# ubc-vision/StableKeypoints

Measured on AMD Instinct MI355X. Metric: images/sec for token-optimization step (SD1.5, 512^2, K=10 kpts), higher is better.
Workload: dtype f32 (fp32 MFMA / VALU throughout; flash attention of the >= 1024-key self-attention layers: 3xbf16 operand split, fp32 accumulate, error <= the fp32 kernel's)

## Files before the change

### include/skp.h

```cpp
#ifndef SKP_H
#define SKP_H

#include <stdint.h>

#ifdef __cplusplus
extern "C" {
#endif

#define SKP_MAX_LAYERS 8
#define SKP_MAX_SUBJECTS 4

#define SKP_E_BADARG (-1)
#define SKP_E_RANGE  (-2)
#define SKP_E_LDS    (-3)

int skp_abi_version(void);

int skp_tune_set(const char* key, int value);
int skp_tune_get(const char* key);

int skp_gemm_nt_f32(const float* A, const float* B, float* C, int M, int N, int K, int Z0, int Z1,
                    int64_t sa0, int64_t sa1, int64_t sam, int64_t sak,
                    int64_t sb0, int64_t sb1, int64_t sbn, int64_t sbk,
                    int64_t sc0, int64_t sc1, int64_t scm, float alpha, void* stream);
// ... 102 lines not shown

int skp_add_layer_norm_ok(int C);
int skp_add_layer_norm_fwd_f32(const float* d, const float* h, const float* gamma, const float* beta, float* x, float* n,
                               float* stat, int64_t rows, int C, float eps, void* stream);
int skp_add_layer_norm_bwd_f32(const float* dn, const float* dskip, const float* x, const float* stat, const float* gamma,
                               float* dx, int64_t rows, int C, void* stream);

int skp_conv3x3_filter_f32(const void* w, void* U, int Cout, int Cin, int flip_transpose, void* stream);
int64_t skp_conv3x3_workspace(int B, int Cin, int Cout, int H, int W, int variant);
int skp_conv3x3_f32(const void* x, const void* U, const void* bias, const void* residual, void* y, void* workspace,
                    int B, int Cin, int Cout, int H, int W, int variant, void* stream);

int skp_conv3x3_f4_filter_f32(const void* w, void* U, int Cout, int Cin, int flip_transpose, void* stream);
int64_t skp_conv3x3_f4_workspace(int B, int Cin, int Cout, int H, int W);
int skp_conv3x3_f4_f32(const void* x, const void* U, const void* bias, const void* residual, void* y, void* workspace,
                       int B, int Cin, int Cout, int H, int W, void* stream);

int skp_conv3x3_f4_stats_blocks(int B, int Cin, int Cout, int H, int W);
int skp_conv3x3_f4_stats_f32(const void* x, const void* U, const void* bias, const void* residual, void* y, float* stats,
                             int B, int Cin, int Cout, int H, int W, void* stream);
int skp_conv3x3_s2_stats_f32(const void* x, const void* U, const void* bias, void* y, float* stats, int B, int Cin, int Cout,
                             int H, int W, int pad, void* stream);
int skp_group_norm_fwd_blocks_f32(const float* x, const float* off, const float* gamma, const float* beta, float* y,
                                  float* mean, float* rstd, const float* bs, int nblk, int pix, int N, int C, int G, int HW,
                                  float eps, int silu, void* stream);

int skp_conv3x3_s2_filter_f32(const void* w, void* U, int Cout, int Cin, void* stream);
int skp_conv3x3_s2_f32(const void* x, const void* U, const void* bias, void* y, int B, int Cin, int Cout, int H, int W,
                       int pad, void* stream);
int64_t skp_conv3x3_s2_workspace(int B, int Cin, int Cout, int H, int W);
int skp_conv3x3_s2_ws_f32(const void* x, const void* U, const void* bias, void* y, void* workspace, int B, int Cin, int Cout,
                          int H, int W, int pad, void* stream);

int skp_conv3x3_small_f32(const void* x, const void* w, const void* bias, void* y, int B, int Cin, int Cout, int H, int W,
                          void* stream);
int skp_conv3x3_small_stats_blocks(int B, int Cin, int Cout, int H, int W);
int skp_conv3x3_small_stats_f32(const void* x, const void* w, const void* bias, void* y, float* stats, int B, int Cin, int Cout,
                                int H, int W, void* stream);

int skp_geglu_fwd_f32(const float* p, float* y, int64_t rows, int inner, void* stream);
int skp_geglu_bwd_f32(const float* p, const float* dy, float* dp, int64_t rows, int inner, void* stream);

int skp_nchw_to_tokens_f32(const float* x, float* y, int B, int C, int HW, void* stream);
int skp_tokens_to_nchw_f32(const float* t, const float* residual, float* y, int B, int C, int HW, void* stream);

int skp_token_stats_f32(const float* M, int T, int R, int num_subjects, float sigma, float eps,
                        int32_t* argmax, float* kl, float* entropy, void* stream);

int skp_select_tokens(const float* kl, const int32_t* argmax_t, int T, int R, int n_cand, int top_k,
                      int64_t* cand, int64_t* sel, void* stream);
int skp_select_tokens_batched(const float* kl, const int32_t* argmax_t, int n, int T, int R, int n_cand, int top_k,
                              int64_t* cand, int64_t* sel, void* stream);

int skp_losses_fwd_f32(const float* M, const float* Mt, const int64_t* sel, int K, int T, int R,
                       const int32_t* argmax, int num_subjects, float sigma,
                       const float* theta_inv , float* partial, float* g_sharp,
                       float* g_eq_a, float* g_eq_b, void* stream);
int skp_losses_fwd_dev_f32(const float* M, const float* Mt, const int64_t* sel, int K, int T, int R,
                           const int32_t* argmax, int num_subjects, float sigma, const float* theta_inv_dev,
                           float* partial, float* g_sharp, float* g_eq_a, float* g_eq_b, void* stream);

int skp_rows_axpy_f32(float* dst, const int64_t* sel, int K, int64_t n, const float* x, const float* a,
                      const float* y, const float* b, void* stream);

#ifdef __cplusplus
}
// ... 3 lines not shown
```

### stablekeypoints_amd/_native.py

```python
from __future__ import annotations

import ctypes as C
import os

import torch

_HERE = os.path.dirname(os.path.abspath(__file__))
LIB_PATH = os.environ.get("SKP_LIB_PATH") or os.path.join(_HERE, "csrc", "libskp_hip.so")
ABI_VERSION = 39

_vp, _i, _f, _i64 = C.c_void_p, C.c_int, C.c_float, C.c_int64

SIGNATURES = {
    "skp_abi_version": [],
    "skp_tune_set": [C.c_char_p, _i],
    "skp_tune_get": [C.c_char_p],
    "skp_group_norm_onepass_ok": [_i, _i, _i, _i],
    "skp_gemm_nt_f32": [_vp, _vp, _vp, _i, _i, _i, _i, _i,
                        _i64, _i64, _i64, _i64, _i64, _i64, _i64, _i64, _i64, _i64, _i64, _f, _vp],
    "skp_qk_logits_f32": [_vp, _vp, _vp, _i, _i, _i, _i, _i, _i, _f, _vp],
    "skp_attn_map_fwd_f32": [C.POINTER(_vp), C.POINTER(_i), _i, _i, _i, _i, _i, _vp, _vp, _vp],
    "skp_attn_map_fwd_ex_f32": [C.POINTER(_vp), C.POINTER(_i), _i, _i, _i, _i, _i, _vp, _vp, _vp, _i, _i64, _i, _vp],
    "skp_attn_map_bwd_ex_f32": [C.POINTER(_vp), C.POINTER(_vp), C.POINTER(_i), _i, _i, _i, _i, _i, _vp, _vp, _vp, _vp,
                                _i, _i64, _i, _vp],
    "skp_attn_map_bwd_workspace": [C.POINTER(_i), _i, _i, _i, _i, _i],
    "skp_attn_map_bwd_f32": [C.POINTER(_vp), C.POINTER(_vp), C.POINTER(_i), _i, _i, _i, _i, _i, _vp, _vp, _vp, _vp],
    "skp_group_norm_coef_f32": [_vp, _vp, _vp, _vp, _vp, _vp, _vp, _vp, _i, _i, _vp, _i, _i, _i, _i, _f, _vp],
    "skp_conv3x3_f4_gn_ok": [_i, _i, _i, _i, _i],
    "skp_conv3x3_f4_gn_f32": [_vp, _vp, _vp, _vp, _vp, _vp, _vp, _i, _i, _i, _i, _i, _vp],
    "skp_unwarp_accumulate_f32": [_vp, _vp, _i, _i, _i, _i, _vp, _vp, _i, _vp],
    "skp_attn_map_fwd_wide_f32": [C.POINTER(_vp), C.POINTER(_i), _i, _i, _i, _i, _i, _vp, _vp, _vp, _i, _i, _vp],
    "skp_attn_map_fwd_wide_ok": [C.POINTER(_i), _i, _i, _i],
    "skp_attn_map_bwd_col_ok": [C.POINTER(_i), _i, _i, _i, _i, _i],
    "skp_attn_map_bwd_col_workspace": [C.POINTER(_i), _i, _i, _i, _i, _i, _i],
    "skp_attn_map_bwd_col_f32": [C.POINTER(_vp), C.POINTER(_vp), C.POINTER(_i), _i, _i, _i, _i, _i, _vp, _vp, _i, _vp, _vp,
                                 _i, _vp],
    "skp_attn_map_bwd_sparse_workspace": [C.POINTER(_i), _i, _i, _i, _i, _i, _i],
    "skp_attn_map_bwd_sparse_f32": [C.POINTER(_vp), C.POINTER(_vp), C.POINTER(_i), _i, _i, _i, _i, _i, _vp, _vp, _i, _vp, _vp,
                                    _i, _vp],
    "skp_token_stats_f32": [_vp, _i, _i, _i, _f, _f, _vp, _vp, _vp, _vp],
    "skp_select_tokens": [_vp, _vp, _i, _i, _i, _i, _vp, _vp, _vp],
    "skp_select_tokens_batched": [_vp, _vp, _i, _i, _i, _i, _i, _vp, _vp, _vp],
# ... 1 lines not shown
    "skp_losses_fwd_dev_f32": [_vp, _vp, _vp, _i, _i, _i, _vp, _i, _f, _vp, _vp, _vp, _vp, _vp, _vp],
    "skp_rows_axpy_f32": [_vp, _vp, _i, _i64, _vp, _vp, _vp, _vp, _vp],
    "skp_cross_attn_fwd_f32": [_vp, _vp, _vp, _vp, _vp, _i, _i, _i, _i, _i, _i, _f, _vp],
    "skp_cross_attn_bwd_workspace": [_i, _i, _i, _i, _i],
    "skp_cross_attn_bwd_f32": [_vp, _vp, _vp, _vp, _vp, _vp, _vp, _vp, _vp, _vp, _i, _i, _i, _i, _i, _i, _f, _vp],
    "skp_group_norm_fwd_f32": [_vp, _vp, _vp, _vp, _vp, _vp, _vp, _vp, _i, _i, _i, _i, _f, _i, _vp],
    "skp_group_norm_bwd_f32": [_vp, _vp, _vp, _vp, _vp, _vp, _vp, _vp, _vp, _i, _i, _i, _i, _f, _i, _vp],
    "skp_group_norm_bwd_add_f32": [_vp, _vp, _vp, _vp, _vp, _vp, _vp, _vp, _vp, _vp, _i, _i, _i, _i, _f, _i, _vp],
    "skp_add_bias_residual_f32": [_vp, _vp, _vp, _vp, _i, _i, _i, _vp],
    "skp_add_layer_norm_ok": [_i],
    "skp_add_layer_norm_fwd_f32": [_vp, _vp, _vp, _vp, _vp, _vp, _vp, _i64, _i, _f, _vp],
    "skp_add_layer_norm_bwd_f32": [_vp, _vp, _vp, _vp, _vp, _vp, _i64, _i, _vp],
    "skp_conv3x3_filter_f32": [_vp, _vp, _i, _i, _i, _vp],
    "skp_conv3x3_workspace": [_i, _i, _i, _i, _i, _i],
    "skp_conv3x3_f32": [_vp, _vp, _vp, _vp, _vp, _vp, _i, _i, _i, _i, _i, _i, _vp],
    "skp_conv3x3_f4_filter_f32": [_vp, _vp, _i, _i, _i, _vp],
    "skp_conv3x3_f4_workspace": [_i, _i, _i, _i, _i],
    "skp_conv3x3_f4_f32": [_vp, _vp, _vp, _vp, _vp, _vp, _i, _i, _i, _i, _i, _vp],
    "skp_flash_attn_fwd_split_ok": [_i, _i, _i, _i, _i, _i],
    "skp_flash_attn_fwd_split_workspace": [_i, _i, _i, _i, _i, _i],
    "skp_flash_attn_fwd_split_f32": [_vp, _vp, _vp, _vp, _vp, _vp, _i, _i, _i, _i, _i, _i, C.c_float, _vp],
    "skp_flash_attn_bwd_split_ok": [_i, _i, _i, _i, _i, _i],
    "skp_flash_attn_bwd_split_workspace": [_i, _i, _i, _i, _i, _i],
    "skp_flash_attn_bwd_split_f32": [_vp, _vp, _vp, _vp, _vp, _vp, _vp, _vp, _vp, _vp, _i, _i, _i, _i, _i, _i, _f, _vp],
    "skp_flash_attn_bwd_split_ld_f32": [_vp, _vp, _vp, _vp, _vp, _vp, _vp, _vp, _vp, _vp, _i, _i, _i, _i, _i, _i, _f, _i, _vp],
    "skp_conv3x3_f4r_ok": [_i, _i, _i, _i, _i],
    "skp_conv3x3_f4r_filter_f32": [_vp, _vp, _i, _i, _i, _vp],
    "skp_conv3x3_f4r_workspace": [_i, _i, _i, _i, _i],
    "skp_conv3x3_f4r_f32": [_vp, _vp, _vp, _vp, _vp, _vp, _i, _i, _i, _i, _i, _vp],
    "skp_conv3x3_s2_filter_f32": [_vp, _vp, _i, _i, _vp],
    "skp_conv3x3_s2_f32": [_vp, _vp, _vp, _vp, _i, _i, _i, _i, _i, _i, _vp],
    "skp_conv3x3_s2_workspace": [_i, _i, _i, _i, _i],
    "skp_conv3x3_s2_ws_f32": [_vp, _vp, _vp, _vp, _vp, _i, _i, _i, _i, _i, _i, _vp],
    "skp_conv3x3_small_f32": [_vp, _vp, _vp, _vp, _i, _i, _i, _i, _i, _vp],
    "skp_conv3x3_small_stats_blocks": [_i, _i, _i, _i, _i],
    "skp_conv3x3_small_stats_f32": [_vp, _vp, _vp, _vp, _vp, _i, _i, _i, _i, _i, _vp],
    "skp_conv3x3_f4_stats_blocks": [_i, _i, _i, _i, _i],
    "skp_conv3x3_f4_stats_f32": [_vp, _vp, _vp, _vp, _vp, _vp, _i, _i, _i, _i, _i, _vp],
    "skp_conv3x3_s2_stats_f32": [_vp, _vp, _vp, _vp, _vp, _i, _i, _i, _i, _i, _i, _vp],
    "skp_group_norm_fwd_blocks_f32": [_vp, _vp, _vp, _vp, _vp, _vp, _vp, _vp, _i, _i, _i, _i, _i, _i, _f, _i, _vp],
    "skp_geglu_fwd_f32": [_vp, _vp, _i64, _i, _vp],
    "skp_geglu_bwd_f32": [_vp, _vp, _vp, _i64, _i, _vp],
    "skp_nchw_to_tokens_f32": [_vp, _vp, _i, _i, _i, _vp],
    "skp_tokens_to_nchw_f32": [_vp, _vp, _vp, _i, _i, _i, _vp],
    "skp_flash_attn_fwd_f32": [_vp, _vp, _vp, _vp, _vp, _i, _i, _i, _i, _i, _i, _f, _vp],
    "skp_flash_attn_bwd_workspace": [_i, _i, _i, _i, _i, _i],
    "skp_flash_attn_bwd_f32": [_vp, _vp, _vp, _vp, _vp, _vp, _vp, _vp, _vp, _vp, _i, _i, _i, _i, _i, _i, _f, _vp],
    "skp_flash_attn_bwd_ld_f32": [_vp, _vp, _vp, _vp, _vp, _vp, _vp, _vp, _vp, _vp, _i, _i, _i, _i, _i, _i, _f, _i, _vp],
    "skp_self_attn_fwd_f32": [_vp, _vp, _vp, _vp, _vp, _i, _i, _i, _i, _f, _vp],
    "skp_self_attn_bwd_f32": [_vp, _vp, _vp, _vp, _vp, _vp, _vp, _vp, _vp, _vp, _i, _i, _i, _i, _f, _vp],
}

_ERR = {-1: "SKP_E_BADARG (null pointer / non-positive size)",
        -2: "SKP_E_RANGE (size outside the built kernel range)",
        -3: "SKP_E_LDS (tile exceeds 160 KiB LDS)"}

_lib = None


class NativeLibraryError(RuntimeError):
    pass


def lib():
    global _lib
    if _lib is not None:
# ... 65 lines not shown
```

### stablekeypoints_amd/csrc/skp_common.h

```cpp
#pragma once
#include <hip/hip_runtime.h>
#include <stdint.h>
#include "../../include/skp.h"

#define SKP_WAVE 64
#define SKP_LOG2E 1.4426950408889634f

typedef float f32x16 __attribute__((ext_vector_type(16)));
typedef float f32x4 __attribute__((ext_vector_type(4)));
typedef float f32x2 __attribute__((ext_vector_type(2)));

enum { SKP_TUNE_WINO_SPLIT = 0, SKP_TUNE_WINO_RAW_MAX_TILES, SKP_TUNE_MAP_BANDS, SKP_TUNE_FA2_TWO_KERNEL_BWD, SKP_TUNE_GN_FOLD_MAX_COUT, SKP_TUNE_CROSS_ATTN_TS,
       SKP_TUNE_COUNT };
int skp_tune(int key);

static inline int skp_launch_status() {
    hipError_t e = hipGetLastError();
    return e == hipSuccess ? 0 : (int)e;
}

__device__ __forceinline__ void skp_cubic_taps(int dst, float ratio, int n, int idx[4], float w[4]) {
    const float A = -0.75f;
    const float src = ratio * ((float)dst + 0.5f) - 0.5f;
    const float fl = floorf(src);
    const float t = src - fl;
    const int i0 = (int)fl;
    float x = t + 1.0f;
    w[0] = ((A * x - 5.0f * A) * x + 8.0f * A) * x - 4.0f * A;
    x = t;
    w[1] = ((A + 2.0f) * x - (A + 3.0f)) * x * x + 1.0f;
    x = 1.0f - t;
    w[2] = ((A + 2.0f) * x - (A + 3.0f)) * x * x + 1.0f;
    x = 2.0f - t;
    w[3] = ((A * x - 5.0f * A) * x + 8.0f * A) * x - 4.0f * A;
#pragma unroll
    for (int i = 0; i < 4; ++i) {
        int v = i0 - 1 + i;
        idx[i] = v < 0 ? 0 : (v > n - 1 ? n - 1 : v);
    }
}

__device__ __forceinline__ float skp_wave_sum(float v) {
#pragma unroll
    for (int o = 32; o > 0; o >>= 1) v += __shfl_xor(v, o, 64);
    return v;
}
// ... 34 lines not shown
```

### stablekeypoints_amd/csrc/skp_select_loss.hip

```cpp
#include "skp_common.h"
#include <string.h>

__device__ __forceinline__ bool skp_better(float v, int i, float bv, int bi) {
    return (v > bv) || (v == bv && i < bi);
}

struct StatsArgs { int T, R, S; float sigma, eps; };

__global__ __launch_bounds__(256) void skp_token_stats_kernel(const float* __restrict__ M, StatsArgs a,
                                                              int32_t* __restrict__ argmax_out,
                                                              float* __restrict__ kl_out, float* __restrict__ ent_out) {
    __shared__ float red_v[4];
    __shared__ int red_i[4];
    __shared__ float red[4];
    __shared__ float s_cy[SKP_MAX_SUBJECTS], s_cx[SKP_MAX_SUBJECTS];
    const int t = blockIdx.x, tid = threadIdx.x, R = a.R, RR = R * R;
    const float* m = M + (size_t)t * RR;
    const float rad = 0.05f * (float)R;
    const float rad2 = rad * rad;
    float maxval0 = 0.f;
    for (int j = 0; j < a.S; ++j) {
        float bv = -INFINITY; int bi = 0x7fffffff;
        for (int p = tid; p < RR; p += 256) {
            const int row = p / R, col = p - row * R;
// ... 338 lines not shown
                                  const int32_t* argmax, int num_subjects, float sigma, const float* theta_inv,
                                  float* partial, float* g_sharp, float* g_eq_a, float* g_eq_b, void* stream) {
    return losses_run(M, Mt, sel, K, T, R, argmax, num_subjects, sigma, theta_inv, nullptr, partial, g_sharp, g_eq_a, g_eq_b, stream);
}

extern "C" int skp_losses_fwd_dev_f32(const float* M, const float* Mt, const int64_t* sel, int K, int T, int R,
                                      const int32_t* argmax, int num_subjects, float sigma, const float* theta_inv_dev,
                                      float* partial, float* g_sharp, float* g_eq_a, float* g_eq_b, void* stream) {
    if (!theta_inv_dev) return SKP_E_BADARG;
    return losses_run(M, Mt, sel, K, T, R, argmax, num_subjects, sigma, nullptr, theta_inv_dev, partial, g_sharp, g_eq_a, g_eq_b, stream);
}

__global__ __launch_bounds__(256) void skp_rows_axpy_kernel(float* __restrict__ dst, const int64_t* __restrict__ sel,
                                                            int64_t n, const float* __restrict__ x,
                                                            const float* __restrict__ a, const float* __restrict__ y,
                                                            const float* __restrict__ b) {
    const int k = blockIdx.y;
    const int64_t i = (int64_t)blockIdx.x * 256 + threadIdx.x;
    if (i >= n) return;
    float v = a[0] * x[(size_t)k * n + i];
    if (y) v += b[0] * y[(size_t)k * n + i];
    dst[(size_t)sel[k] * n + i] += v;
}

extern "C" int skp_rows_axpy_f32(float* dst, const int64_t* sel, int K, int64_t n, const float* x, const float* a,
                                 const float* y, const float* b, void* stream) {
    if (!dst || !sel || !x || !a || K <= 0 || n <= 0 || (y && !b)) return SKP_E_BADARG;
    if (K > 65535) return SKP_E_RANGE;
    hipLaunchKernelGGL(skp_rows_axpy_kernel, dim3((unsigned)((n + 255) / 256), K), dim3(256), 0, (hipStream_t)stream,
                       dst, sel, n, x, a, y, b);
    return skp_launch_status();
}

extern "C" int skp_abi_version(void) { return 39; }

static int g_tune[SKP_TUNE_COUNT] = {0};
static const char* const g_tune_names[SKP_TUNE_COUNT] = {"wino_split", "wino_raw_max_tiles", "map_bands", "fa2_two_kernel_bwd", "gn_fold_max_cout", "cross_attn_ts"};
int skp_tune(int key) { return (key >= 0 && key < SKP_TUNE_COUNT) ? g_tune[key] : 0; }
extern "C" int skp_tune_set(const char* key, int value) {
    if (!key || value < 0) return SKP_E_BADARG;
    for (int i = 0; i < SKP_TUNE_COUNT; ++i)
        if (!strcmp(key, g_tune_names[i])) { g_tune[i] = value; return 0; }
    return SKP_E_RANGE;
}
extern "C" int skp_tune_get(const char* key) {
    if (!key) return SKP_E_BADARG;
    for (int i = 0; i < SKP_TUNE_COUNT; ++i)
        if (!strcmp(key, g_tune_names[i])) return g_tune[i];
    return SKP_E_RANGE;
}
```

### stablekeypoints_amd/ops.py

```python
from __future__ import annotations

import contextlib
import weakref
from typing import List, Sequence, Tuple

import torch

from . import _native as N
from . import routes


def _stream() -> int:
    return torch.cuda.current_stream().cuda_stream


def _dev(t: torch.Tensor, name: str) -> torch.Tensor:
    if not t.is_cuda:
        raise RuntimeError(f"{name}: the StableKeypoints hot path runs on the HIP kernels only "
                           f"(got a {t.device} tensor; there is no CPU fallback)")
    if t.dtype != torch.float32:
        raise RuntimeError(f"{name}: expected float32, got {t.dtype}")
    return t if t.is_contiguous() else t.contiguous()


# ... 794 lines not shown
    def backward(ctx, gx, gn):
        x, stat, weight = ctx.saved_tensors
        C = x.shape[-1]
        if gn is None:
            dx = gx
        else:
            gn = _dev(gn, "gn")
            gx = _dev(gx, "gx") if gx is not None else None
            dx = torch.empty_like(x)
            N.check(N.lib().skp_add_layer_norm_bwd_f32(gn.data_ptr(), gx.data_ptr() if gx is not None else None, x.data_ptr(),
                                                       stat.data_ptr(), weight.data_ptr(), dx.data_ptr(), x.numel() // C, C,
                                                       _stream()), "skp_add_layer_norm_bwd_f32")
        return (dx if ctx.has_d else None), dx, None, None, None


def add_layer_norm(d, h, norm: torch.nn.LayerNorm):
    routes.note("add_layer_norm", "add_ln")
    return AddLayerNormFn.apply(d, h, norm.weight, norm.bias, norm.eps)


def conv3x3_supported(x_shape, w_shape, need_grad=True):
    if len(w_shape) != 4 or tuple(w_shape[2:]) != (3, 3) or len(x_shape) != 4:
        return False
    co, ci = int(w_shape[0]), int(w_shape[1])
    if co % 32 or ci % 32:
        return False
    _, _, h, w = (int(v) for v in x_shape)
    return max(ci * h * w, co * h * w, 16 * ci * co) * 4 < 2 ** 31


_FILTER_FORMS = {"f2": ("skp_conv3x3_filter_f32", 16),
                 "f4": ("skp_conv3x3_f4_filter_f32", 36),
                 "f4r": ("skp_conv3x3_f4r_filter_f32", 9),
                 "s2": ("skp_conv3x3_s2_filter_f32", 9)}


def _filters(weight, form, backward=False):
    def build():
        w = _dev(weight.detach(), "weight")
        co, ci = w.shape[:2]
        name, per_pair = _FILTER_FORMS[form]
        U = torch.empty(per_pair * co * ci, device=w.device, dtype=torch.float32)
        if form == "s2":
            N.check(N.lib().skp_conv3x3_s2_filter_f32(w.data_ptr(), U.data_ptr(), co, ci, _stream()), name)
        else:
            N.check(getattr(N.lib(), name)(w.data_ptr(), U.data_ptr(), *((ci, co, 1) if backward else (co, ci, 0)), _stream()), name)
        return U
    return cached(weight, ("filters", form, bool(backward)), (weight,), build)


def _wino_filters(weight, backward):
    return _filters(weight, "f2", backward)


def _wino4_filters(weight, backward):
    return _filters(weight, "f4", backward)


def _wino4r_filters(weight, backward):
    return _filters(weight, "f4r", backward)


def _conv3x3_raw(x, U, bias, cout, variant=0, split=True, residual=None, out=None):
    B, ci, H, W = x.shape
    y = out if out is not None else torch.empty(B, cout, H, W, device=x.device, dtype=torch.float32)
    ws = _workspace("skp_conv3x3_workspace", B, ci, cout, H, W, int(variant), device=x.device) if split else None
    N.check(N.lib().skp_conv3x3_f32(x.data_ptr(), U.data_ptr(), _ptr(bias), _ptr(residual), y.data_ptr(), _ptr(ws),
                                    B, ci, cout, H, W, int(variant), _stream()), "skp_conv3x3_f32")
    return y


def _conv3x3_f4_raw(x, U, bias, cout, split=True, residual=None, out=None, stats=None):
    B, ci, H, W = x.shape
    y = out if out is not None else torch.empty(B, cout, H, W, device=x.device, dtype=torch.float32)
    if stats is not None:
        N.check(N.lib().skp_conv3x3_f4_stats_f32(x.data_ptr(), U.data_ptr(), _ptr(bias), _ptr(residual), y.data_ptr(),
                                                 stats.data_ptr(), B, ci, cout, H, W, _stream()), "skp_conv3x3_f4_stats_f32")
# ... 352 lines not shown
        ctx.weight = weight
        ctx.xshape, ctx.pad = tuple(x.shape), int(pad)
        return _conv3x3_s2_raw(x, weight, bias, pad, False)

    @staticmethod
    def backward(ctx, dy):
        w = ctx.weight
        b, c, h, wd = ctx.xshape
        co = w.shape[0]
        if S2_BWD_OWN and h % 2 == 0 and wd % 2 == 0 and conv3x3_wanted((b, co, h, wd), (c, co, 3, 3)):
            dy = _dev(dy, "dy")
            routes.note("conv3x3_s2.bwd_data", "zero_stuffed")
            up = torch.zeros(b, co, h, wd, device=dy.device, dtype=torch.float32)
            o = 0 if ctx.pad == 1 else 1
            up[:, :, o::2, o::2] = dy
            return _conv3x3_run(up, w, True, None, None, c), None, None, None
        routes.note("conv3x3_s2.bwd_data", "lib")
        if ctx.pad == 1:
            return torch.nn.grad.conv2d_input(ctx.xshape, w, dy.contiguous(), stride=2, padding=1), None, None, None
        dxp = torch.nn.grad.conv2d_input((b, c, h + 1, wd + 1), w, dy.contiguous(), stride=2, padding=0)
        return dxp[:, :, :h, :wd], None, None, None


def conv3x3_s2(x, weight, bias=None, pad: int = 0, want_stats: bool = False):
    if weight.requires_grad or (bias is not None and bias.requires_grad):
        raise RuntimeError("conv3x3_s2: frozen weights only")
    if torch.is_grad_enabled() and x.requires_grad:
        return ConvS2Fn.apply(x, weight, bias, int(pad))
    return _conv3x3_s2_raw(x, weight, bias, pad, want_stats)


def _conv3x3_s2_raw(x, weight, bias, pad, want_stats):
    x = _dev(x.detach(), "x")
    routes.note("conv3x3_s2", "s2_direct")
    U = _filters(weight, "s2")
    B, ci, H, W = x.shape
    co = weight.shape[0]
    y = torch.empty(B, co, H // 2, W // 2, device=x.device, dtype=torch.float32)
    if want_stats and GN_FUSED_STATS:
        nblk = (H // 16) * (W // 32)
        stats = torch.empty(B, co, nblk, 2, device=x.device, dtype=torch.float32)
        N.check(N.lib().skp_conv3x3_s2_stats_f32(x.data_ptr(), U.data_ptr(), _ptr(bias), y.data_ptr(), stats.data_ptr(),
                                                 B, ci, co, H, W, int(pad), _stream()), "skp_conv3x3_s2_stats_f32")
        y._skp_blocks = (stats, nblk, 128)
        return y
    ws = _workspace("skp_conv3x3_s2_workspace", B, ci, co, H, W, device=x.device)
    N.check(N.lib().skp_conv3x3_s2_ws_f32(x.data_ptr(), U.data_ptr(), _ptr(bias), y.data_ptr(), _ptr(ws), B, ci, co, H, W,
                                          int(pad), _stream()), "skp_conv3x3_s2_ws_f32")
    return y


class GEGLUFn(torch.autograd.Function):

    @staticmethod
    def forward(ctx, proj):
        proj = _dev(proj, "proj")
        inner = proj.shape[-1] // 2
        rows = proj.numel() // (2 * inner)
        y = torch.empty(*proj.shape[:-1], inner, device=proj.device, dtype=torch.float32)
        N.check(N.lib().skp_geglu_fwd_f32(proj.data_ptr(), y.data_ptr(), rows, inner, _stream()), "skp_geglu_fwd_f32")
        ctx.save_for_backward(proj)
        return y

    @staticmethod
    def backward(ctx, dy):
        (proj,) = ctx.saved_tensors
        dy = _dev(dy, "dy")
        inner = proj.shape[-1] // 2
        dp = torch.empty_like(proj)
        N.check(N.lib().skp_geglu_bwd_f32(proj.data_ptr(), dy.data_ptr(), dp.data_ptr(), proj.numel() // (2 * inner), inner,
                                          _stream()), "skp_geglu_bwd_f32")
# ... 57 lines not shown
```

### stablekeypoints_amd/routes.py

```python
from __future__ import annotations

import contextlib
import threading
from typing import Dict, Iterable, Optional, Tuple

KINDS = ("hip", "library", "eager", "host")

_WINO = {"wino4_c128": "hip", "wino4_c64": "hip", "wino4_raw": "hip", "wino2": "hip", "lib": "library"}
_FLASH = {"flash_split": "hip", "flash_f32": "hip", "self_attn_gen1": "hip"}
_BLOCK = {"fused": "hip", "eager": "eager"}

ROUTES: Dict[str, Dict[str, str]] = {
    "conv3x3": dict(_WINO),
    "conv3x3.bwd_data": dict(_WINO),
    "conv_in": {"small": "hip"},
    "conv_out": {"lib": "library"},
    "conv3x3_s2": {"s2_direct": "hip"},
    "conv3x3_s2.bwd_data": {"zero_stuffed": "hip", "lib": "library"},
    "downsample": {"s2_direct": "hip", "eager": "eager"},
    "downsample.untiled": {"eager": "eager"},
    "resnet": dict(_BLOCK),
    "transformer2d": dict(_BLOCK),
    "transformer_block": dict(_BLOCK),
    "time_embedding": {"eager": "eager"},
    "group_norm": {"gn_fold": "hip", "gn_apply": "hip"},
    "group_norm.stats": {"producer_blocks": "hip", "own_pass": "hip"},
    "add_layer_norm": {"add_ln": "hip"},
    "vae.attention": {"lib_core": "library", "eager": "eager"},
    "vae.tail": {"composed": "hip", "eager": "eager"},
    "attn.cross": {"ca_token_split": "hip", "ca_plain": "hip", "flash": "hip", "host": "host"},
    "attn.self": {"fused_qkv": "hip", "plain": "hip", "host": "host"},
    "flash.fwd": dict(_FLASH),
    "flash.bwd": dict(_FLASH),
    "map.fwd": {"map_fused": "hip", "map_wide": "hip", "map_groups": "hip", "host": "host"},
    "map.bwd": {"map_dense": "hip", "map_dense_groups": "hip", "map_col": "hip", "map_tok": "hip"},
    "map.select": {"batched": "hip", "per_image": "hip"},
    "map.collect": {"reference_ops": "library", "host": "host"},
    "select.rank": {"select_kernel": "hip", "sort": "library"},
}

DOCUMENTED_LIBRARY_ROUTES: Dict[Tuple[str, str], str] = {
    ("vae.attention", "lib_core"): "VAE mid-block attention, one head of d = 512: baddbmm + softmax + bmm (no flash kernel at that head size)",
    ("conv_out", "lib"): "UNet conv_out 320 -> 4 (full forward only) and a VAE conv_out 512 -> 8 whose tail is not composed: "
                         "output channels below the Winograd kernels' 32-channel blocks",
    ("downsample.untiled", "eager"): "Downsample2D whose input is no multiple of the stride-2 kernel's 16 x 32 pixel tile (SD-1.5 at 512^2: "
                                     "1280 -> 1280 at 16^2 -> 8^2): the module's own stride-2 convolution on MIOpen, forward and backward",
}


class UnexpectedRoute(RuntimeError):
# ... 141 lines not shown
```

Measured before the change: 52.88.

## Add Winograd-based stride-2 3x3 convolution kernel for downsample layers

Adds a new stride-2 3x3 convolution path that splits the filter into four polyphase sub-kernels. Each sub-kernel is computed with a Winograd-style 5x5 transform using fp32 MFMA, a persistent grid, a ring of prefetched filter loads, and optional fused GroupNorm statistics. It replaces the direct stride-2 kernel for eligible shapes (Cin>=128, enough tiles, pad==0) and aims to reduce multiply work in the downsample convs. The cost is extra transform arithmetic, a larger filter workspace, and some numerical error from the transforms.

Result: faster. 53.68 (median of 6 runs) (+1.5%).

```diff
diff --git a/include/skp.h b/include/skp.h
--- a/include/skp.h
+++ b/include/skp.h
@@ -158,6 +158,13 @@
 int skp_conv3x3_s2_ws_f32(const void* x, const void* U, const void* bias, void* y, void* workspace, int B, int Cin, int Cout,
                           int H, int W, int pad, void* stream);
 
+int skp_conv3x3_s2w_ok(int B, int Cin, int Cout, int H, int W, int pad);
+int skp_conv3x3_s2w_filter_f32(const void* w, void* U, int Cout, int Cin, int pad, void* stream);
+int skp_conv3x3_s2w_f32(const void* x, const void* U, const void* bias, void* y, int B, int Cin, int Cout, int H, int W,
+                        int pad, void* stream);
+int skp_conv3x3_s2w_stats_f32(const void* x, const void* U, const void* bias, void* y, float* stats, int B, int Cin, int Cout,
+                              int H, int W, int pad, void* stream);
+
 int skp_conv3x3_small_f32(const void* x, const void* w, const void* bias, void* y, int B, int Cin, int Cout, int H, int W,
                           void* stream);
 int skp_conv3x3_small_stats_blocks(int B, int Cin, int Cout, int H, int W);
diff --git a/stablekeypoints_amd/_native.py b/stablekeypoints_amd/_native.py
--- a/stablekeypoints_amd/_native.py
+++ b/stablekeypoints_amd/_native.py
@@ -7,7 +7,7 @@
 
 _HERE = os.path.dirname(os.path.abspath(__file__))
 LIB_PATH = os.environ.get("SKP_LIB_PATH") or os.path.join(_HERE, "csrc", "libskp_hip.so")
-ABI_VERSION = 39
+ABI_VERSION = 40
 
 _vp, _i, _f, _i64 = C.c_void_p, C.c_int, C.c_float, C.c_int64
 
@@ -75,6 +75,10 @@
     "skp_conv3x3_s2_f32": [_vp, _vp, _vp, _vp, _i, _i, _i, _i, _i, _i, _vp],
     "skp_conv3x3_s2_workspace": [_i, _i, _i, _i, _i],
     "skp_conv3x3_s2_ws_f32": [_vp, _vp, _vp, _vp, _vp, _i, _i, _i, _i, _i, _i, _vp],
+    "skp_conv3x3_s2w_ok": [_i, _i, _i, _i, _i, _i],
+    "skp_conv3x3_s2w_filter_f32": [_vp, _vp, _i, _i, _i, _vp],
+    "skp_conv3x3_s2w_f32": [_vp, _vp, _vp, _vp, _i, _i, _i, _i, _i, _i, _vp],
+    "skp_conv3x3_s2w_stats_f32": [_vp, _vp, _vp, _vp, _vp, _i, _i, _i, _i, _i, _i, _vp],
     "skp_conv3x3_small_f32": [_vp, _vp, _vp, _vp, _i, _i, _i, _i, _i, _vp],
     "skp_conv3x3_small_stats_blocks": [_i, _i, _i, _i, _i],
     "skp_conv3x3_small_stats_f32": [_vp, _vp, _vp, _vp, _vp, _i, _i, _i, _i, _i, _vp],
diff --git a/stablekeypoints_amd/csrc/skp_common.h b/stablekeypoints_amd/csrc/skp_common.h
--- a/stablekeypoints_amd/csrc/skp_common.h
+++ b/stablekeypoints_amd/csrc/skp_common.h
@@ -11,7 +11,7 @@
 typedef float f32x2 __attribute__((ext_vector_type(2)));
 
 enum { SKP_TUNE_WINO_SPLIT = 0, SKP_TUNE_WINO_RAW_MAX_TILES, SKP_TUNE_MAP_BANDS, SKP_TUNE_FA2_TWO_KERNEL_BWD, SKP_TUNE_GN_FOLD_MAX_COUT, SKP_TUNE_CROSS_ATTN_TS,
-       SKP_TUNE_COUNT };
+       SKP_TUNE_CONV_S2W, SKP_TUNE_COUNT };
 int skp_tune(int key);
 
 static inline int skp_launch_status() {
diff --git a/stablekeypoints_amd/csrc/skp_conv_s2w.hip b/stablekeypoints_amd/csrc/skp_conv_s2w.hip
--- /dev/null
+++ b/stablekeypoints_amd/csrc/skp_conv_s2w.hip
@@ -0,0 +1,362 @@
+#include <algorithm>
+#include "skp_common.h"
+#include "skp_wino4_common.h"
+#include <stdlib.h>
+
+namespace {
+
+#ifdef S2W_ALL_BLOCKS
+constexpr bool S2W_SKIP = false;
+#else
+constexpr bool S2W_SKIP = true;
+#endif
+
+constexpr int s2w_rp(int k) { return k >> 1; }
+constexpr int s2w_cp(int k) { return 1 - (k & 1); }
+constexpr int s2w_ni(int k) { return (S2W_SKIP && s2w_rp(k)) ? 4 : 5; }
+constexpr int s2w_nj(int k) { return (S2W_SKIP && s2w_cp(k)) ? 4 : 5; }
+constexpr int s2w_np(int k) { return s2w_ni(k) * s2w_nj(k); }
+constexpr int s2w_e0(int k) { return k == 0 ? 0 : s2w_e0(k - 1) + s2w_np(k - 1); }
+constexpr int S2W_NE = s2w_e0(3) + s2w_np(3);
+constexpr int S2W_RING = S2W_SKIP ? 9 : 10;
+constexpr int S2W_D = 6;
+constexpr int S2W_STAGE_F4 = 25 * 4 * 16;
+static_assert(S2W_NE % S2W_RING == 0 && S2W_D < S2W_RING, "ring");
+
+__global__ void skp_s2w_filter_kernel(const float* __restrict__ w, float* __restrict__ U, int Cout, int Cin) {
+    const int idx = blockIdx.x * blockDim.x + threadIdx.x;
+    if (idx >= Cout * Cin) return;
+    const int co = idx / Cin, ci = idx - co * Cin;
+    const float* p = w + ((size_t)co * Cin + ci) * 9;
+    const double G[5][2] = {{0.5, 0.0}, {-0.5, -0.5}, {-1.0 / 6, 1.0 / 6}, {1.0 / 6, 1.0 / 3}, {0.0, 1.0}};
+    const int c16 = ci >> 4, kq = (ci >> 2) & 3, m = ci & 3;
+    float* dst = U + ((((size_t)c16 * S2W_NE) * 4 + kq) * Cout + co) * 4 + m;
+    const size_t blk = (size_t)16 * Cout;
+#pragma unroll
+    for (int k = 0; k < 4; ++k) {
+        const int rp = s2w_rp(k), cp = s2w_cp(k);
+        double g[2][2];
+#pragma unroll
+        for (int a = 0; a < 2; ++a)
+#pragma unroll
+            for (int b = 0; b < 2; ++b) {
+                const bool nz = (rp == 0 || a == 0) && (cp == 0 || b == 0);
+                const int ra = rp == 0 ? 2 * a : 1, cb = cp == 0 ? 2 * b : 1;
+                g[a][b] = nz ? (double)p[ra * 3 + cb] : 0.0;
+            }
+        double t[5][2];
+#pragma unroll
+        for (int i = 0; i < 5; ++i)
+#pragma unroll
+            for (int b = 0; b < 2; ++b) t[i][b] = G[i][0] * g[0][b] + G[i][1] * g[1][b];
+        int e = s2w_e0(k);
+#pragma unroll
+        for (int i = 0; i < 5; ++i)
+#pragma unroll
+            for (int j = 0; j < 5; ++j) {
+                if (i >= s2w_ni(k) || j >= s2w_nj(k)) continue;
+                dst[(size_t)e * blk] = (float)(t[i][0] * G[j][0] + t[i][1] * G[j][1]);
+                ++e;
+            }
+    }
+}
+
+template <int N, class T>
+__device__ __forceinline__ void s2w_in1d(const T (&d)[5], T (&t)[5]) {
+    const T a = d[3] - d[1];
+    t[0] = 2.f * (d[0] - d[2]) + a;
+    t[1] = a - (d[1] + d[2]);
+    t[2] = 3.f * (d[1] - d[2]) + a;
+    t[3] = a;
+    if (N == 5) t[4] = (d[4] - d[2]) - 2.f * a;
+}
+__device__ __forceinline__ void s2w_out1d(const float (&m)[5], float (&y)[4]) {
+    const float s12 = m[1] + m[2], d12 = m[1] - m[2];
+    y[0] = m[0] + s12 + m[3];
+    y[1] = d12 + 2.f * m[3];
+    y[2] = s12 + 4.f * m[3];
+    y[3] = d12 + 8.f * m[3] + m[4];
+}
+
+template <int P, int CB>
+__device__ __forceinline__ void s2w_mfma(float a, float b) {
+    asm volatile("v_mfma_f32_16x16x4_f32 a[%0:%1], %2, %3, a[%0:%1]" : : "n"(4 * (2 * P + CB)), "n"(4 * (2 * P + CB) + 3), "v"(a), "v"(b) : W4_AGPR_CLOBBERS);
+}
+
+template <bool STATS>
+__global__ __launch_bounds__(256, 1) void skp_s2w_conv_kernel(Wino4Args a) {
+    extern __shared__ f32x4 vst[];
+    f32x2* const sst = (f32x2*)(vst + 2 * S2W_STAGE_F4);
+    const int tid = threadIdx.x, lane = tid & 63, wave = __builtin_amdgcn_readfirstlane(tid >> 6);
+    const int i16 = lane & 15, kq = lane >> 4;
+    const int HW = a.H * a.W, OH = a.H >> 1, OW = a.W >> 1, OHW = OH * OW;
+    int tblock, cg, zsplit;
+    int wid = blockIdx.x;
+    while (wid < a.vtotal && !w4_work(a, wid, tblock, cg, zsplit)) wid += gridDim.x;
+    if (wid >= a.vtotal) return;
+
+    const int tl = tid & 15, tc = tid >> 4;
+    int vA, vC, vA8, vC8;
+    auto aim_transform = [&](int tb, bool valid) {
+        const int tg = tb * 16 + tl;
+        const bool tv = valid && tg < a.nTiles;
+        const int tgc = tv ? tg : 0;
+        const int b = tgc / a.tilesPerImg, rem = tgc - b * a.tilesPerImg;
+        const int ty = rem / a.tilesX, tx = rem - ty * a.tilesX;
+        const int pbase = (((b * a.Cin + tc) * a.H + 8 * ty) * a.W + 8 * tx) * 4;
+        const bool r8 = 8 * ty + 8 < a.H, c8 = 8 * tx + 8 < a.W;
+        vA = tv ? pbase : SKP_OOB;
+        vC = (tv && c8) ? pbase + 32 : SKP_OOB;
+        vA8 = (tv && r8) ? pbase : SKP_OOB;
+        vC8 = (tv && r8 && c8) ? pbase + 32 : SKP_OOB;
+    };
+    aim_transform(tblock, true);
+    const i32x4 xrs = skp_make_rsrc(a.x, a.x_bytes);
+    const i32x4 urs = skp_make_rsrc(a.U, a.u_bytes);
+    const i32x4 brs = skp_make_rsrc(a.bias, a.bias ? (unsigned)a.Cout * 4u : 0u);
+    const i32x4 yrs = skp_make_rsrc(a.y, a.y_bytes);
+    f32x2 d[5][5];
+    auto load_row = [&](int cin0, int rp, int k) {
+        const int row = 2 * k + rp;
+        const int so = (cin0 * HW + row * a.W) * 4;
+        const int va = row >= 8 ? vA8 : vA, vc = row >= 8 ? vC8 : vC;
+        const f32x4 m0 = skp_buf_load_f32x4(xrs, va, so, 0);
+        const f32x4 m1 = skp_buf_load_f32x4(xrs, va + 16, so, 0);
+        const float c8 = skp_buf_load_f32(xrs, vc, so, 0);
+        d[k][0] = f32x2{m0[0], m0[1]};
+        d[k][1] = f32x2{m0[2], m0[3]};
+        d[k][2] = f32x2{m1[0], m1[1]};
+        d[k][3] = f32x2{m1[2], m1[3]};
+        d[k][4] = f32x2{c8, 0.f};
+    };
+    auto col_pass = [&](int c, auto ni_c) {
+        constexpr int NI = decltype(ni_c)::value;
+        f32x2 v[5], t[5];
+#pragma unroll
+        for (int i = 0; i < 5; ++i) v[i] = d[i][c];
+        s2w_in1d<NI>(v, t);
+#pragma unroll
+        for (int i = 0; i < NI; ++i) d[i][c] = t[i];
+    };
+    auto row_pass_store = [&](int buf, int i, int cp, auto nj_c) {
+        constexpr int NJ = decltype(nj_c)::value;
+        float r[5] = {d[i][0][cp], d[i][1][cp], d[i][2][cp], d[i][3][cp], d[i][4][cp]};
+        float t[5];
+        s2w_in1d<NJ>(r, t);
+        float* dst = (float*)(vst + buf * S2W_STAGE_F4) + (((i * NJ) * 4 + (tc >> 2)) * 16 + tl) * 4 + (tc & 3);
+#pragma unroll
+        for (int j = 0; j < NJ; ++j) dst[j * (4 * 16 * 4)] = t[j];
+    };
+
+    {
+        constexpr int NI = s2w_ni(0), NJ = s2w_nj(0);
+#pragma unroll
+        for (int k = 0; k < NI; ++k) load_row(0, 0, k);
+#pragma unroll
+        for (int c = 0; c < 5; ++c) col_pass(c, std::integral_constant<int, NI>{});
+#pragma unroll
+        for (int i = 0; i < NI; ++i) row_pass_store(0, i, s2w_cp(0), std::integral_constant<int, NJ>{});
+    }
+
+    const int u_blk = 4 * a.Cout * 16;
+    const int nsteps = a.total_steps;
+
+    for (;;) {
+        const int tile0 = tblock * 16;
+        const int n0 = (cg * 4 + wave) * 32;
+        int uvo[2];
+#pragma unroll
+        for (int cb = 0; cb < 2; ++cb) uvo[cb] = (kq * a.Cout + n0 + cb * 16 + i16) * 16;
+        f32x4 ua[S2W_RING][2];
+#pragma unroll
+        for (int q = 0; q < S2W_D; ++q)
+#pragma unroll
+            for (int cb = 0; cb < 2; ++cb) ua[q][cb] = skp_buf_load_f32x4(urs, uvo[cb], q * u_blk, 0);
+
+        int wnext = wid + gridDim.x, tb_n = 0, cg_n = 0, z_n = 0;
+        while (wnext < a.vtotal && !w4_work(a, wnext, tb_n, cg_n, z_n)) wnext += gridDim.x;
+        const bool has_next = wnext < a.vtotal;
+
+        w4_unroll([&](auto rc) { asm volatile("v_accvgpr_write_b32 a[%0], 0" : : "n"(decltype(rc)::value) : W4_AGPR_CLOBBERS); },
+                  std::make_integer_sequence<int, 200>{});
+        __syncthreads();
+
+        auto run_group = [&](int s, auto mode_c) {
+            constexpr int MODE = decltype(mode_c)::value;
+            const int ub = s * S2W_NE * u_blk;
+            w4_unroll([&](auto kc) {
+                constexpr int k = decltype(kc)::value, kn = (k + 1) & 3;
+                constexpr int NJ = s2w_nj(k), NP = s2w_np(k), E0 = s2w_e0(k);
+                constexpr int NIn = s2w_ni(kn), NJn = s2w_nj(kn);
+                constexpr bool heavy = (k & 1) == 1;
+                if (MODE == 1 && k == 3) aim_transform(tb_n, has_next);
+                const int cin_side = k == 1 ? s * 16 : (MODE == 0 ? (s + 1) * 16 : 0);
+                const f32x4* vb = vst + (k & 1) * S2W_STAGE_F4 + kq * 16 + i16;
+                f32x4 va[3];
+                va[0] = vb[0];
+                va[1] = vb[64];
+                w4_unroll([&](auto ec) {
+                    constexpr int e = decltype(ec)::value, p = 5 * (e / NJ) + (e % NJ);
+                    {
+                        constexpr int q = E0 + e + S2W_D;
+                        if (MODE == 0 || q < S2W_NE) {
+#pragma unroll
+                            for (int cb = 0; cb < 2; ++cb) ua[q % S2W_RING][cb] = skp_buf_load_f32x4(urs, uvo[cb], ub + q * u_blk, 0);
+                        }
+                    }
+                    if constexpr (heavy && e < NIn) load_row(cin_side, s2w_rp(kn), e);
+                    else if constexpr (heavy && e >= NP - NIn - 5 && e < NP - NIn) col_pass(e - (NP - NIn - 5), std::integral_constant<int, NIn>{});
+                    else if constexpr (e >= NP - NIn) row_pass_store((k + 1) & 1, e - (NP - NIn), s2w_cp(kn), std::integral_constant<int, NJn>{});
+                    if (e + 2 < NP) va[(e + 2) % 3] = vb[(e + 2) * 64];
+                    w4_unroll([&](auto mc) {
+                        constexpr int m = decltype(mc)::value;
+                        s2w_mfma<p, 0>(ua[(E0 + e) % S2W_RING][0][m], va[e % 3][m]);
+                        s2w_mfma<p, 1>(ua[(E0 + e) % S2W_RING][1][m], va[e % 3][m]);
+                    }, std::make_integer_sequence<int, 4>{});
+                    __builtin_amdgcn_sched_barrier(0);
+                }, std::make_integer_sequence<int, NP>{});
+                if (!(MODE == 1 && k == 3)) __syncthreads();
+            }, std::make_integer_sequence<int, 4>{});
+        };
+        for (int s = 0; s + 1 < nsteps; ++s) run_group(s, std::integral_constant<int, 0>{});
+        run_group(nsteps - 1, std::integral_constant<int, 1>{});
+
+        int o_base;
+        bool t_ok;
+        {
+            const int tg = tile0 + i16;
+            t_ok = tg < a.nTiles;
+            const int tgc = t_ok ? tg : 0;
+            const int b = tgc / a.tilesPerImg, rem = tgc - b * a.tilesPerImg;
+            const int ty = rem / a.tilesX, tx = rem - ty * a.tilesX;
+            o_base = ((b * a.Cout) * OH + 4 * ty) * OW + 4 * tx;
+        }
+        float bvs[8];
+#pragma unroll
+        for (int e = 0; e < 8; ++e) bvs[e] = skp_buf_load_f32(brs, (n0 + (e >> 2) * 16 + 4 * kq + (e & 3)) * 4, 0, 0);
+        asm volatile("s_nop 15\n\ts_nop 15" ::: "memory");
+        __builtin_amdgcn_sched_barrier(0);
+        w4_unroll([&](auto ec) {
+            constexpr int e = decltype(ec)::value, cb = e >> 2, r = e & 3;
+            const int co = n0 + cb * 16 + 4 * kq + r;
+            const int vo = (o_base + co * OHW) * 4;
+            const float bv = bvs[e];
+            float t[5][4];
+            w4_unroll([&](auto ic) {
+                constexpr int i = decltype(ic)::value;
+                float m[5];
+                w4_unroll([&](auto jc) { constexpr int j = decltype(jc)::value; m[j] = w4_acc_read<4 * (2 * (5 * i + j) + cb) + r>(); },
+                          std::make_integer_sequence<int, 5>{});
+                s2w_out1d(m, t[i]);
+            }, std::make_integer_sequence<int, 5>{});
+            f32x4 o[4];
+#pragma unroll
+            for (int ox = 0; ox < 4; ++ox) {
+                float m[5], yv[4];
+#pragma unroll
+                for (int i = 0; i < 5; ++i) m[i] = t[i][ox];
+                s2w_out1d(m, yv);
+#pragma unroll
+                for (int oy = 0; oy < 4; ++oy) o[oy][ox] = yv[oy] + bv;
+            }
+#pragma unroll
+            for (int oy = 0; oy < 4; ++oy) skp_buf_store_f32x4(o[oy], yrs, t_ok ? vo + oy * OW * 4 : SKP_OOB, 0, 0);
+            if (STATS) w4_park_stats(sst, wave * 8 + e, lane, o, t_ok);
+            __builtin_amdgcn_sched_barrier(0);
+        }, std::make_integer_sequence<int, 8>{});
+        if (STATS) {
+            __syncthreads();
+            if (tid < 128) {
+                const int wv = tid >> 5, lc = tid & 31;
+                w4_store_stats(a, sst, wv * 8 + ((lc >> 4) << 2) + (lc & 3), (lc >> 2) & 3, tile0, (cg * 4 + wv) * 32 + lc);
+            }
+        }
+        if (!has_next) break;
+        wid = wnext; tblock = tb_n; cg = cg_n; zsplit = z_n;
+    }
+}
+
+static bool s2w_layout_ok(int B, int Cin, int Cout, int H, int W, int pad) {
+    if (B <= 0 || Cin <= 0 || Cout <= 0 || H <= 0 || W <= 0 || pad != 0) return false;
+    if ((Cin % 16) || (Cout % 128) || (H % 8) || (W % 8)) return false;
+    const unsigned long long xb = (unsigned long long)B * Cin * H * W * 4, ub = (unsigned long long)S2W_NE * Cin * Cout * 4,
+                             yb = (unsigned long long)B * Cout * (H / 2) * (W / 2) * 4;
+    return xb < 0x80000000ull && ub < 0x80000000ull && yb < 0x80000000ull;
+}
+
+static bool s2w_shape_ok(int B, int Cin, int Cout, int H, int W) {
+    const long long units = (((long long)B * (H / 8) * (W / 8) + 15) / 16) * (Cout / 128);
+    return Cin >= 128 && units >= 256;
+}
+
+}
+
+extern "C" int skp_conv3x3_s2w_ok(int B, int Cin, int Cout, int H, int W, int pad) {
+    if (!s2w_layout_ok(B, Cin, Cout, H, W, pad)) return 0;
+    const int force = skp_tune(SKP_TUNE_CONV_S2W);
+    if (force) return force == 1 ? 1 : 0;
+    return s2w_shape_ok(B, Cin, Cout, H, W) ? 1 : 0;
+}
+
+extern "C" int skp_conv3x3_s2w_filter_f32(const void* w, void* U, int Cout, int Cin, int pad, void* stream) {
+    if (!w || !U || Cout <= 0 || Cin <= 0 || (pad != 0 && pad != 1)) return SKP_E_BADARG;
+    if ((Cin & 15) || (unsigned long long)S2W_NE * Cin * Cout * 4 >= 0x80000000ull) return SKP_E_RANGE;
+    const int n = Cout * Cin;
+    hipLaunchKernelGGL(skp_s2w_filter_kernel, dim3((n + 255) / 256), dim3(256), 0, (hipStream_t)stream, (const float*)w, (float*)U,
+                       Cout, Cin);
+    return skp_launch_status();
+}
+
+static int s2w_run(const void* x, const void* U, const void* bias, void* y, float* stats, int B, int Cin, int Cout, int H, int W,
+                   int pad, void* stream) {
+    if (!x || !U || !y || B <= 0 || Cin <= 0 || Cout <= 0 || H <= 0 || W <= 0 || (pad != 0 && pad != 1)) return SKP_E_BADARG;
+    if (!s2w_layout_ok(B, Cin, Cout, H, W, pad)) return SKP_E_RANGE;
+    Wino4Args a = {};
+    a.x = (const float*)x; a.U = (const float*)U; a.bias = (const float*)bias; a.y = (float*)y;
+    a.B = B; a.Cin = Cin; a.Cout = Cout; a.H = H; a.W = W;
+    a.tilesX = W / 8;
+    a.tilesPerImg = a.tilesX * (H / 8);
+    a.nTiles = B * a.tilesPerImg;
+    if (stats && (a.tilesPerImg % 16)) return SKP_E_RANGE;
+    a.x_bytes = (unsigned)((size_t)B * Cin * H * W * 4);
+    a.u_bytes = (unsigned)((size_t)S2W_NE * Cin * Cout * 4);
+    a.y_bytes = (unsigned)((size_t)B * Cout * (H / 2) * (W / 2) * 4);
+    a.total_steps = a.steps = Cin / 16;
+    a.splits = 1;
+    a.stats = stats;
+    a.sblk = a.tilesPerImg / 16;
+    a.ntb = (a.nTiles + 15) / 16;
+    a.ncg = Cout / 128;
+    a.tb_per_xcd = a.ntb >= 64 ? (a.ntb + 7) / 8 : 0;
+    a.gx = a.tb_per_xcd ? 8 * a.tb_per_xcd * a.ncg : 8 * ((a.ncg + 7) / 8) * a.ntb;
+    a.vtotal = a.gx;
+    const size_t lds = (size_t)2 * S2W_STAGE_F4 * sizeof(f32x4) + 32 * 64 * sizeof(f32x2);
+    static bool attr_set = false;
+    if (!attr_set) {
+        hipError_t e = hipFuncSetAttribute((const void*)skp_s2w_conv_kernel<false>, hipFuncAttributeMaxDynamicSharedMemorySize, (int)lds);
+        if (e != hipSuccess) return (int)e;
+        e = hipFuncSetAttribute((const void*)skp_s2w_conv_kernel<true>, hipFuncAttributeMaxDynamicSharedMemorySize, (int)lds);
+        if (e != hipSuccess) return (int)e;
+        attr_set = true;
+    }
+    static const int persist = [] {
+        int dev = 0, ncu = 0;
+        if (hipGetDevice(&dev) != hipSuccess || hipDeviceGetAttribute(&ncu, hipDeviceAttributeMultiprocessorCount, dev) != hipSuccess) ncu = 256;
+        return ncu;
+    }();
+    const dim3 grid((unsigned)(persist >= 8 ? std::min(a.vtotal, persist & ~7) : a.vtotal), 1, 1);
+    if (stats) hipLaunchKernelGGL(skp_s2w_conv_kernel<true>, grid, dim3(256), lds, (hipStream_t)stream, a);
+    else hipLaunchKernelGGL(skp_s2w_conv_kernel<false>, grid, dim3(256), lds, (hipStream_t)stream, a);
+    return skp_launch_status();
+}
+
+extern "C" int skp_conv3x3_s2w_f32(const void* x, const void* U, const void* bias, void* y, int B, int Cin, int Cout, int H, int W,
+                                   int pad, void* stream) {
+    return s2w_run(x, U, bias, y, nullptr, B, Cin, Cout, H, W, pad, stream);
+}
+
+extern "C" int skp_conv3x3_s2w_stats_f32(const void* x, const void* U, const void* bias, void* y, float* stats, int B, int Cin,
+                                         int Cout, int H, int W, int pad, void* stream) {
+    if (!stats) return SKP_E_BADARG;
+    return s2w_run(x, U, bias, y, stats, B, Cin, Cout, H, W, pad, stream);
+}
diff --git a/stablekeypoints_amd/csrc/skp_select_loss.hip b/stablekeypoints_amd/csrc/skp_select_loss.hip
--- a/stablekeypoints_amd/csrc/skp_select_loss.hip
+++ b/stablekeypoints_amd/csrc/skp_select_loss.hip
@@ -394,10 +394,10 @@
     return skp_launch_status();
 }
 
-extern "C" int skp_abi_version(void) { return 39; }
+extern "C" int skp_abi_version(void) { return 40; }
 
 static int g_tune[SKP_TUNE_COUNT] = {0};
-static const char* const g_tune_names[SKP_TUNE_COUNT] = {"wino_split", "wino_raw_max_tiles", "map_bands", "fa2_two_kernel_bwd", "gn_fold_max_cout", "cross_attn_ts"};
+static const char* const g_tune_names[SKP_TUNE_COUNT] = {"wino_split", "wino_raw_max_tiles", "map_bands", "fa2_two_kernel_bwd", "gn_fold_max_cout", "cross_attn_ts", "conv_s2w"};
 int skp_tune(int key) { return (key >= 0 && key < SKP_TUNE_COUNT) ? g_tune[key] : 0; }
 extern "C" int skp_tune_set(const char* key, int value) {
     if (!key || value < 0) return SKP_E_BADARG;
diff --git a/stablekeypoints_amd/ops.py b/stablekeypoints_amd/ops.py
--- a/stablekeypoints_amd/ops.py
+++ b/stablekeypoints_amd/ops.py
@@ -850,7 +850,8 @@
 _FILTER_FORMS = {"f2": ("skp_conv3x3_filter_f32", 16),
                  "f4": ("skp_conv3x3_f4_filter_f32", 36),
                  "f4r": ("skp_conv3x3_f4r_filter_f32", 9),
-                 "s2": ("skp_conv3x3_s2_filter_f32", 9)}
+                 "s2": ("skp_conv3x3_s2_filter_f32", 9),
+                 "s2w": ("skp_conv3x3_s2w_filter_f32", 81)}
 
 
 def _filters(weight, form, backward=False):
@@ -861,6 +862,8 @@
         U = torch.empty(per_pair * co * ci, device=w.device, dtype=torch.float32)
         if form == "s2":
             N.check(N.lib().skp_conv3x3_s2_filter_f32(w.data_ptr(), U.data_ptr(), co, ci, _stream()), name)
+        elif form == "s2w":
+            N.check(N.lib().skp_conv3x3_s2w_filter_f32(w.data_ptr(), U.data_ptr(), co, ci, 0, _stream()), name)
         else:
             N.check(getattr(N.lib(), name)(w.data_ptr(), U.data_ptr(), *((ci, co, 1) if backward else (co, ci, 0)), _stream()), name)
         return U
@@ -1279,11 +1282,24 @@
 
 def _conv3x3_s2_raw(x, weight, bias, pad, want_stats):
     x = _dev(x.detach(), "x")
-    routes.note("conv3x3_s2", "s2_direct")
-    U = _filters(weight, "s2")
     B, ci, H, W = x.shape
     co = weight.shape[0]
     y = torch.empty(B, co, H // 2, W // 2, device=x.device, dtype=torch.float32)
+    if N.lib().skp_conv3x3_s2w_ok(B, ci, co, H, W, int(pad)):
+        routes.note("conv3x3_s2", "s2_wino")
+        U = _filters(weight, "s2w")
+        nblk = (H // 8) * (W // 8) // 16
+        if want_stats and GN_FUSED_STATS and nblk * 16 == (H // 8) * (W // 8):
+            stats = torch.empty(B, co, nblk, 2, device=x.device, dtype=torch.float32)
+            N.check(N.lib().skp_conv3x3_s2w_stats_f32(x.data_ptr(), U.data_ptr(), _ptr(bias), y.data_ptr(), stats.data_ptr(),
+                                                      B, ci, co, H, W, int(pad), _stream()), "skp_conv3x3_s2w_stats_f32")
+            y._skp_blocks = (stats, nblk, 256)
+            return y
+        N.check(N.lib().skp_conv3x3_s2w_f32(x.data_ptr(), U.data_ptr(), _ptr(bias), y.data_ptr(), B, ci, co, H, W, int(pad),
+                                            _stream()), "skp_conv3x3_s2w_f32")
+        return y
+    routes.note("conv3x3_s2", "s2_direct")
+    U = _filters(weight, "s2")
     if want_stats and GN_FUSED_STATS:
         nblk = (H // 16) * (W // 32)
         stats = torch.empty(B, co, nblk, 2, device=x.device, dtype=torch.float32)
diff --git a/stablekeypoints_amd/routes.py b/stablekeypoints_amd/routes.py
--- a/stablekeypoints_amd/routes.py
+++ b/stablekeypoints_amd/routes.py
@@ -15,7 +15,7 @@
     "conv3x3.bwd_data": dict(_WINO),
     "conv_in": {"small": "hip"},
     "conv_out": {"lib": "library"},
-    "conv3x3_s2": {"s2_direct": "hip"},
+    "conv3x3_s2": {"s2_direct": "hip", "s2_wino": "hip"},
     "conv3x3_s2.bwd_data": {"zero_stuffed": "hip", "lib": "library"},
     "downsample": {"s2_direct": "hip", "eager": "eager"},
     "downsample.untiled": {"eager": "eager"},
```
